# marcinmiklitz/pywindow

Hardware: AMD Instinct MI355X
Metric: trajectory frames/sec full_analysis (pore+windows), CC3 1k-frame (higher is better)
Workload: dtype f64

## Files before the change

### pywindow_amd/csrc/pw_lbfgsb.hpp

```cpp
#pragma once
#include "pw_blas.hpp"
#include "pw_team.hpp"

#if defined(PW_PROFILE) && defined(__HIP_DEVICE_COMPILE__)
#define LB_T0(var) long long var = wall_clock64()
#define LB_T1(slot, var) do { if (prof && T::lane() == 0) atomicAdd(&prof[slot], (unsigned long long)(wall_clock64() - var)); } while (0)
#else
#define LB_T0(var) do {} while (0)
#define LB_T1(slot, var) do {} while (0)
#endif
#if defined(PW_PROFILE) && defined(PW_LB_FINE) && defined(__HIP_DEVICE_COMPILE__)
#define LB_F0(var) long long var = clock64()
#define LB_F1(slot, var) do { if (prof && T::lane() == 0) atomicAdd(&prof[slot], (unsigned long long)(clock64() - var)); } while (0)
#define LB_M0(var) long long var = clock64()
#define LB_M1(slot, var) do { if (m->prof_fine && T::lane() == 0) atomicAdd(&m->prof_fine[slot], (unsigned long long)(clock64() - var)); } while (0)
#else
#define LB_F0(var) do {} while (0)
#define LB_F1(slot, var) do {} while (0)
#define LB_M0(var) do {} while (0)
#define LB_M1(slot, var) do {} while (0)
#endif

namespace pw {

enum LbTask : int {
    LB_START = 0,
    LB_NEW_X = 1,
    LB_FG = 3,
    LB_CONVERGENCE = 4,
    LB_STOP = 5,
    LB_WARNING = 6,
    LB_ERROR = 7,
    LB_ABNORMAL = 8,
};
enum LbMsg : int {
    LBM_NONE = 0,
    LBM_FG_START = 301,
    LBM_FG_LNSRCH = 302,
    LBM_CONV_PGTOL = 401,
    LBM_CONV_FTOL = 402,
};

constexpr int LB_M = 10;

struct LsState {
    double ginit, gtest, gx, gy, finit, fx, fy, stx, sty, stmin, stmax, width, width1;
    int brackt, stage;
};

template <int N>
struct LbMem {
    static constexpr int M = LB_M;
    static constexpr int M2 = 2 * LB_M;
    double l[N], u[N];
    double x[N], g[N];
    double ws[M * N], wy[M * N];
    double sy[M * M], ss[M * M], wt[M * M];
    double wn[M2 * M2], wn1d[M2];
    double z[N], r[N], d[N], t[N], xp[N];
    double wa[8 * M];
    double acc[2 * M];
    double dsy[M], rsy[M], sqy[M], rsq[M], rwt[M], rwn[M2];
    double iwn[M];
    double tri[64];
    int pair[64];
    double le[N], ue[N];
    LsState ls;
#if defined(PW_PROFILE) && defined(PW_LB_FINE)
    unsigned long long* prof_fine;
#endif
    int cand[32];
    int nbd[N];
    int index[N], iwhere[N], indx2[N];
};

template <class T>
PW_NOINLINE PW_HD inline void lb_trsv_un_wave(int n, const double* a, int lda, double* x) {
    PW_ASSUME_LDS(a);
    PW_ASSUME_LDS(x);
    const int lane = T::lane();
    double xk = lane < n ? x[lane] : 0.0;
    for (int i = n - 1; i >= 0; --i) {
        const double* ci = a + (long)i * lda;
        double xi = T::bcast_u(xk, i) / ci[i];
        if (lane == i) xk = xi;
        if (lane < i) xk = pw_fma(-xi, ci[lane], xk);
    }
    T::wave_sync();
    if (lane < n) x[lane] = xk;
    T::wave_sync();
}
template <class T>
PW_NOINLINE PW_HD inline void lb_trsv_ut_wave(int n, const double* a, int lda, double* x) {
    PW_ASSUME_LDS(a);
    PW_ASSUME_LDS(x);
    const int lane = T::lane();
    const double* ci = a + (long)(lane < n ? lane : 0) * lda;
    double xk = lane < n ? x[lane] : 0.0;
    double ak = 0.0;
    for (int s = 0; s < n; ++s) {
        double xs = T::bcast_u(xk, s);
        if (s > 0) xs = xs - T::bcast_u(ak, s);
        xs = xs / a[s + (long)s * lda];
        if (lane == s) xk = xs;
        if (lane > s && lane < n) {
            if (lane >= 16 && s < 16) {
                if (s == 15) {
                    double sl[4];
                    for (int l = 0; l < 4; ++l) {
                        double a0 = ci[l] * T::bcast_u(xk, l);
                        double a1 = ci[4 + l] * T::bcast_u(xk, 4 + l);
                        double a2 = ci[8 + l] * T::bcast_u(xk, 8 + l);
                        double a3 = ci[12 + l] * T::bcast_u(xk, 12 + l);
                        sl[l] = ((a0 + a1) + a2) + a3;
                    }
                    ak = (sl[0] + sl[2]) + (sl[1] + sl[3]);
                }
            } else {
                ak = pw_fma(xs, ci[s], ak);
            }
        }
    }
    T::wave_sync();
    if (lane < n) x[lane] = xk;
    T::wave_sync();
}


#if defined(__HIP_DEVICE_COMPILE__)
typedef DeviceTeam<1> LbWave;
__device__ inline int lb_uniform(int v) { return __builtin_amdgcn_readfirstlane(v); }
template <class P>
__device__ inline P* lb_uniform(P* p) {
    union { P* p; int i[2]; } a;
    a.p = p;
    a.i[0] = __builtin_amdgcn_readfirstlane(a.i[0]);
    a.i[1] = __builtin_amdgcn_readfirstlane(a.i[1]);
    return a.p;
}
template <class T, int NMAX, bool SPEC>
__device__ inline __attribute__((always_inline)) double lb_solve_ut_reg(int n, const double* a, int lda, const double* rdiag,
                                                                       double xk, double* tnum) {
    PW_ASSUME_LDS(a);
    PW_ASSUME_LDS(rdiag);
    const int lane = T::lane();
    const bool act = lane < n;
    const int li = act ? lane : 0;
    const double* ci = a + li * lda;
    double c[NMAX];
#pragma unroll
    for (int k = 0; k < NMAX; ++k) c[k] = ci[k];
    int dli = li * (lda + 1);
    asm volatile("" : "+v"(dli));
    double dg = a[dli], rd = rdiag[li];
    if (!act) { dg = 1.0; rd = 1.0; xk = 0.0; }
    const double x0 = xk;
    double ak = 0.0;
#pragma unroll
    for (int s = 0; s < NMAX; ++s) {
        if (s >= n) continue;
        const double mine = SPEC ? pw_div_ru(xk - ak, dg, rd) : pw_div_r(xk - ak, dg, rd);
        const double xs = T::bcast_u(mine, s);
        xk = lane == s ? xs : xk;
        if (NMAX > 16 && s < 16) {
            if (s == 15) {
                double sl[4];
#pragma unroll
                for (int l = 0; l < 4; ++l) {
                    double a0 = c[l] * T::bcast_u(xk, l);
                    double a1 = c[4 + l] * T::bcast_u(xk, 4 + l);
                    double a2 = c[8 + l] * T::bcast_u(xk, 8 + l);
                    double a3 = c[12 + l] * T::bcast_u(xk, 12 + l);
                    sl[l] = ((a0 + a1) + a2) + a3;
                }
                const double blk = (sl[0] + sl[2]) + (sl[1] + sl[3]);
                ak = (act && lane >= 16) ? blk : ak;
            }
            ak = (act && lane > s && lane < 16) ? pw_fma(xs, c[s], ak) : ak;
        } else {
            ak = (act && lane > s) ? pw_fma(xs, c[s], ak) : ak;
        }
    }
    if (SPEC) *tnum = act ? x0 - ak : 1.0;
    return xk;
}
template <class T, int NMAX, bool SPEC>
__device__ inline __attribute__((always_inline)) double lb_solve_un_reg(int n, const double* a, int lda, const double* rdiag,
                                                                       double xk, double* tnum) {
    PW_ASSUME_LDS(a);
    PW_ASSUME_LDS(rdiag);
    const int lane = T::lane();
    const bool act = lane < n;
    const int li = act ? lane : 0;
    double rw[NMAX];
#pragma unroll
    for (int i = 0; i < NMAX; ++i) rw[i] = a[li + i * lda];
    int dli = li * (lda + 1);
    asm volatile("" : "+v"(dli));
    double dg = a[dli], rd = rdiag[li];
    if (!act) { dg = 1.0; rd = 1.0; xk = 0.0; }
    double tn = 1.0;
#pragma unroll
    for (int i = NMAX - 1; i >= 0; --i) {
        if (i >= n) continue;
        const double mine = SPEC ? pw_div_ru(xk, dg, rd) : pw_div_r(xk, dg, rd);
        const double xi = T::bcast_u(mine, i);
        if (SPEC) tn = lane == i ? xk : tn;
        xk = lane == i ? xi : xk;
        xk = lane < i ? pw_fma(-xi, rw[i], xk) : xk;
    }
    if (SPEC) *tnum = tn;
    return xk;
}
__device__ inline unsigned lb_expo(double x) {
    union { double d; unsigned long long u; } c;
    c.d = x;
    return (unsigned)(c.u >> 32) & 0x7ff00000u;
}
__device__ inline bool lb_plain_range(unsigned emin, unsigned emax) {
    return (emin - 0x2bc00000u) <= 0x2bc00000u && (emax - 0x2bc00000u) <= 0x2bc00000u;
}

template <class T, int N, bool SPEC>
__device__ inline __attribute__((always_inline)) int lb_bmv_body(LbMem<N>* m, int col, const double* v, double* p) {
    constexpr int M = LB_M;
    const int lane = T::lane();
    const bool act = lane < col;
    const int li = act ? lane : 0;
    {
        const unsigned long long z = T::ballot(act && m->wt[li + M * li] == 0.0);
        if (z) return (int)__builtin_ctzll(z) + 1;
    }
    LB_M0(tb0);
    const double vi = act ? v[li] : 0.0, vc = act ? v[col + li] : 0.0;
    unsigned emin = 0x3ff00000u, emax = 0x3ff00000u;
    const int pk = m->pair[lane];
    const int pa_ = pk & 0xff, pb_ = (pk >> 8) & 0xff;
    const bool pact = pa_ < col;
    const int sa = pact ? pa_ : 1, sb = pact ? pb_ : 0;
    const double sy_ab = m->sy[sa + M * sb], d_b = m->dsy[sb], r_b = m->rsy[sb];
    {
        const double num = pact ? sy_ab * v[sb] : 1.0;
        if (SPEC) {
            const unsigned e = lb_expo(num);
            emin = e < emin ? e : emin;
            emax = e > emax ? e : emax;
        }
        const double term = SPEC ? pw_div_ru(num, d_b, r_b) : pw_div_r(num, d_b, r_b);
        m->tri[lane] = term;
    }
    T::wave_sync();
    double sum = 0.0;
    {
        const int base = li * (li - 1) / 2;
        double q[M - 1];
#pragma unroll
        for (int k = 0; k < M - 1; ++k) q[k] = m->tri[(base + k) & 63];
#pragma unroll
        for (int k = 0; k < M - 1; ++k) {
            const bool on = act && k < lane && k + 1 < col;
            sum = sum + (on ? q[k] : 0.0);
        }
    }
    double xk = lane == 0 ? vc : vc + sum;
    double t_ut = 1.0, t_un = 1.0;
    LB_M1(3, tb0);
    LB_M0(tb1);
    xk = lb_solve_ut_reg<T, M, SPEC>(col, m->wt, M, m->rwt, xk, &t_ut);
    LB_M1(4, tb1);
    LB_M0(tb2);
    const double sq = act ? m->sqy[li] : 1.0, rs = act ? m->rsq[li] : 1.0;
    const double pa = SPEC ? pw_div_ru(vi, sq, rs) : pw_div_r(vi, sq, rs);
    xk = lb_solve_un_reg<T, M, SPEC>(col, m->wt, M, m->rwt, xk, &t_un);
    LB_M1(5, tb2);
    LB_M0(tb3);
    const double pi = SPEC ? pw_div_ru(-pa, sq, rs) : pw_div_r(-pa, sq, rs);
    if (act) p[col + lane] = xk;
    T::wave_sync();
    {
        const double num = pact ? sy_ab * p[col + sa] : 1.0;
        if (SPEC) {
            const unsigned e = lb_expo(num);
            emin = e < emin ? e : emin;
            emax = e > emax ? e : emax;
        }
        const double term = SPEC ? pw_div_ru(num, d_b, r_b) : pw_div_r(num, d_b, r_b);
        m->tri[lane] = term;
    }
    T::wave_sync();
    double sum2 = 0.0;
    {
        double q[M];
#pragma unroll
        for (int k = 1; k < M; ++k) q[k] = m->tri[(k * (k - 1) / 2 + li) & 63];
#pragma unroll
        for (int k = 1; k < M; ++k) {
            const bool on = act && k > lane && k < col;
            sum2 = sum2 + (on ? q[k] : 0.0);
        }
    }
    if (SPEC) {
        unsigned e;
        e = lb_expo(t_ut); emin = e < emin ? e : emin; emax = e > emax ? e : emax;
        e = lb_expo(t_un); emin = e < emin ? e : emin; emax = e > emax ? e : emax;
        if (act) {
            e = lb_expo(vi); emin = e < emin ? e : emin; emax = e > emax ? e : emax;
            e = lb_expo(pa); emin = e < emin ? e : emin; emax = e > emax ? e : emax;
        }
        bool good = lb_plain_range(emin, emax) && rs != 0.0 && (!pact || r_b != 0.0) && (!act || m->rwt[li] != 0.0);
        if (T::ballot(!good)) return -1;
    }
    if (act) p[lane] = pi + sum2;
    T::wave_sync();
    LB_M1(6, tb3);
    return 0;
}
template <class T, int N>
PW_NOINLINE __device__ inline int lb_bmv_wave_guarded(LbMem<N>* m, int col, const double* v, double* p) {
    m = lb_uniform(m); v = lb_uniform(v); p = lb_uniform(p); col = lb_uniform(col);
    PW_ASSUME_LDS(m);
    PW_ASSUME_LDS(v);
    PW_ASSUME_LDS(p);
    return lb_bmv_body<T, N, false>(m, col, v, p);
// ... 1132 lines not shown
            WN1(iy, jy) = WN1(iy, jy) + temp1 - temp3;
            WN1(is, js) = WN1(is, js) - temp2 + temp4;
        }
        for (int e = T::lane(); e < upcl * upcl; e += T::WSIZE) {
            int ii = e / upcl, jy = e % upcl;
            int is = M + ii;
            int ipntr = (head + ii) % M, jpntr = (head + jy) % M;
            double temp1 = 0.0, temp3 = 0.0;
            for (int k = 0; k < nenter; ++k) {
                int k1 = indx2[k];
                temp1 = temp1 + WS(ipntr)[k1] * WY(jpntr)[k1];
            }
            for (int k = ileave - 1; k < N; ++k) {
                int k1 = indx2[k];
                temp3 = temp3 + WS(ipntr)[k1] * WY(jpntr)[k1];
            }
            if (is <= jy + M) WN1(is, jy) = WN1(is, jy) + temp1 - temp3;
            else WN1(is, jy) = WN1(is, jy) - temp1 + temp3;
        }
        }
        T::wave_sync();
        for (int e = T::lane(); e < col * col; e += T::WSIZE) {
            int iy = e / col, jy = e % col;
            int is = col + iy, is1 = M + iy;
            if (jy <= iy) {
                int js = col + jy, js1 = M + jy;
                double w = WN1(iy, jy) / theta;
                if (jy == iy) w = w + SY(iy, iy);
                WN(jy, iy) = w;
                WN(js, is) = WN1(is1, js1) * theta;
            }
            if (jy < iy) WN(jy, is) = -WN1(is1, jy);
            else WN(jy, is) = WN1(is1, jy);
        }
        T::wave_sync();
        LB_F1(8, fk1);
        if (col <= 2) {
            LB_F0(fks);
            const int rs = formk_tail_small<T>();
            LB_F1(9, fks);
            return rs;
        }
        LB_F0(fk2);
        int inf = factor<T>(2);
        LB_F1(9, fk2);
        if (inf != 0) return -1;
        int col2 = 2 * col;
        LB_F0(fk3);
#if defined(__HIP_DEVICE_COMPILE__)
        inf = p_dtrtrs_u<T>(true, col, col, wn, M2, &WN(0, col), M2, T::WSIZE == 64 ? mem->iwn : (const double*)nullptr);
#else
        inf = p_dtrtrs_u<T>(true, col, col, wn, M2, &WN(0, col), M2);
#endif
        LB_F1(10, fk3);
        LB_F0(fk4);
        for (int e = T::lane(); e < col * col; e += T::WSIZE) {
            int is = col + e / col, js = col + e % col;
            if (js < is) continue;
            WN(is, js) = WN(is, js) + b_ddot(col, &WN(0, is), &WN(0, js));
        }
        T::wave_sync();
        inf = factor<T>(3);
        LB_F1(11, fk4);
        (void)col2;
        if (inf != 0) return -2;
        return 0;
    }

    template <class T>
    PW_HD int cmprlb() {
        PW_ASSUME_LDS(mem);
        if (!cnstnd && col > 0) {
            for (int i = 0; i < N; ++i) r[i] = -g[i];
        } else {
            for (int i = 0; i < nfree; ++i) {
                int k = index[i];
                r[i] = -theta * (z[k] - x[k]) - g[k];
            }
            T::wave_sync();
            int inf = bmv<T>(wa + 2 * M, wa);
            if (inf != 0) return -8;
            LB_F0(fr);
#if defined(__HIP_DEVICE_COMPILE__)
            if (T::WSIZE == 64) {
                const int lj = T::lane();
                const bool lon = lj < col;
                const int pj = (head + (lon ? lj : 0)) % M;
                const double a1 = lon ? wa[lj] : 0.0, a2 = lon ? theta * wa[col + lj] : 0.0;
                double t1[N], t2[N], rl[N];
                for (int i = 0; i < N; ++i) {
                    const int k = i < nfree ? index[i] : 0;
                    t1[i] = WY(pj)[k] * a1;
                    t2[i] = WS(pj)[k] * a2;
                    rl[i] = r[i];
                }
#pragma unroll
                for (int jj = 0; jj < M; ++jj) {
                    if (jj >= col) continue;
#pragma unroll
                    for (int i = 0; i < N; ++i)
                        if (i < nfree) rl[i] = rl[i] + T::bcast_u(t1[i], jj) + T::bcast_u(t2[i], jj);
                }
                T::wave_sync();
                for (int i = 0; i < N; ++i)
                    if (i < nfree) r[i] = rl[i];
                T::wave_sync();
            } else
#endif
            {
                int pointr = head;
                for (int j = 0; j < col; ++j) {
                    double a1 = wa[j];
                    double a2 = theta * wa[col + j];
                    for (int i = 0; i < nfree; ++i) {
                        int k = index[i];
                        r[i] = r[i] + WY(pointr)[k] * a1 + WS(pointr)[k] * a2;
                    }
                    pointr = (pointr + 1) % M;
                }
            }
            LB_F1(13, fr);
        }
        return 0;
    }

    template <class T>
    PW_HD int subsm() {
        PW_ASSUME_LDS(mem);
        const int nsub = nfree;
        double* wv = wa;
        double* dd = r;
        double* xs = z;
        if (nsub <= 0) return 0;
        T::wave_sync();
        LB_F0(fsh);
        for (int i = T::lane(); i < col; i += T::WSIZE) {
            int pi = (head + i) % M;
            double temp1 = 0.0, temp2 = 0.0;
            for (int j = 0; j < nsub; ++j) {
                int k = index[j];
                temp1 = temp1 + WY(pi)[k] * dd[j];
                temp2 = temp2 + WS(pi)[k] * dd[j];
            }
            wv[i] = temp1;
            wv[col + i] = theta * temp2;
        }
        T::wave_sync();
        LB_F1(29, fsh);
        int col2 = 2 * col;
        LB_F0(fs1);
        int inf;
        if (col <= 2) {
            inf = subsm_solves_small<T>(wv);
        } else
#if defined(__HIP_DEVICE_COMPILE__)
        if (T::WSIZE == 64) {
            inf = lb_subsm_solves_wave<LbWave, N>(mem, col, wv);
        } else
#endif
        {
            inf = p_dtrtrs_u<T>(true, col2, 1, wn, M2, wv, col2);
            if (inf != 0) return inf;
            for (int i = T::lane(); i < col; i += T::WSIZE) wv[i] = -wv[i];
            T::wave_sync();
            inf = p_dtrtrs_u<T>(false, col2, 1, wn, M2, wv, col2);
        }
        LB_F1(12, fs1);
        if (inf != 0) return inf;
        LB_F0(fst);
        if (T::WSIZE == 64 && col * nsub <= 32) {
            const int t = T::lane();
            const int nsu = T::uniform_i(nsub), cu = T::uniform_i(col);
            const int jy_ = nsu == 3 ? t / 3 : (nsu == 2 ? t >> 1 : t), i_ = t - jy_ * nsu;
            const double rth = 1.0 / theta;
            if (jy_ < cu) {
                const int pj = (head + jy_) % M, k = index[i_];
                mem->tri[t] = WY(pj)[k] * wv[jy_] / theta;
                mem->tri[32 + t] = WS(pj)[k] * wv[cu + jy_];
            }
            double acc_[N];
            for (int i = 0; i < N; ++i) acc_[i] = dd[i < nsu ? i : 0];
            T::wave_sync();
            double q1[M * N], q2[M * N];
#pragma unroll
            for (int jy = 0; jy < M; ++jy)
#pragma unroll
                for (int i = 0; i < N; ++i) {
                    const int at = (jy * nsu + i) & 31;
                    q1[jy * N + i] = mem->tri[at];
                    q2[jy * N + i] = mem->tri[32 + at];
                }
#pragma unroll
            for (int jy = 0; jy < M; ++jy)
#pragma unroll
                for (int i = 0; i < N; ++i) {
                    const bool on = jy < cu && i < nsu;
                    acc_[i] = acc_[i] + (on ? q1[jy * N + i] : -0.0) + (on ? q2[jy * N + i] : -0.0);
                }
            T::wave_sync();
            for (int i = 0; i < N; ++i)
                if (i < nsu) dd[i] = rth * acc_[i];
            T::wave_sync();
        } else {
            int pointr = head;
            for (int jy = 0; jy < col; ++jy) {
                int js = col + jy;
                for (int i = 0; i < nsub; ++i) {
                    int k = index[i];
                    dd[i] = dd[i] + WY(pointr)[k] * wv[jy] / theta + WS(pointr)[k] * wv[js];
                }
                pointr = (pointr + 1) % M;
            }
            b_dscal(nsub, 1.0 / theta, dd);
        }
        iword = 0;
        b_dcopy(N, xs, xp);
        {
            int kk[N], nb[N];
            double dk[N], xk[N], lk[N], uk[N];
            for (int i = 0; i < N; ++i) {
                const bool on = i < nsub;
                kk[i] = on ? index[i] : 0;
            }
            for (int i = 0; i < N; ++i) {
                dk[i] = dd[i < nsub ? i : 0]; xk[i] = xs[kk[i]]; nb[i] = nbd[kk[i]]; lk[i] = l[kk[i]]; uk[i] = u[kk[i]];
            }
            T::wave_sync();
            for (int i = 0; i < N; ++i) {
                if (i >= nsub) continue;
                double nx;
                bool hit = false;
                if (nb[i] != 0) {
                    nx = xk[i];
                    if (nb[i] == 1) {
                        nx = pw_max(lk[i], xk[i] + dk[i]);
                        hit = nx == lk[i];
                    } else if (nb[i] == 2) {
                        nx = pw_min(uk[i], pw_max(lk[i], xk[i] + dk[i]));
                        hit = nx == lk[i] || nx == uk[i];
                    } else if (nb[i] == 3) {
                        nx = pw_min(uk[i], xk[i] + dk[i]);
                        hit = nx == uk[i];
                    }
                } else {
                    nx = xk[i] + dk[i];
                }
                if (hit) iword = 1;
                xs[kk[i]] = nx;
            }
            T::wave_sync();
        }
        LB_F1(30, fst);
        if (iword == 0) return 0;
        double dd_p = 0.0;
        for (int i = 0; i < N; ++i) dd_p = dd_p + (xs[i] - x[i]) * g[i];
        if (dd_p > 0.0) {
            b_dcopy(N, xp, xs);
            double alpha = 1.0;
            double temp1 = alpha;
            int ibd = 0;
            for (int i = 0; i < nsub; ++i) {
                int k = index[i];
                double dk = dd[i];
                if (nbd[k] != 0) {
                    if (dk < 0.0 && nbd[k] <= 2) {
                        double temp2 = l[k] - xs[k];
                        if (temp2 >= 0.0) temp1 = 0.0;
                        else if (dk * alpha < temp2) temp1 = temp2 / dk;
                    } else if (dk > 0.0 && nbd[k] >= 2) {
                        double temp2 = u[k] - xs[k];
                        if (temp2 <= 0.0) temp1 = 0.0;
                        else if (dk * alpha > temp2) temp1 = temp2 / dk;
                    }
                    if (temp1 < alpha) {
                        alpha = temp1;
                        ibd = i;
                    }
                }
            }
            if (alpha < 1.0) {
                double dk = dd[ibd];
                int k = index[ibd];
                if (dk > 0.0) {
                    xs[k] = u[k];
                    dd[ibd] = 0.0;
                } else if (dk < 0.0) {
                    xs[k] = l[k];
                    dd[ibd] = 0.0;
                }
            }
            for (int i = 0; i < nsub; ++i) {
                int k = index[i];
                xs[k] = xs[k] + alpha * dd[i];
            }
        }
        return 0;
    }

    template <class T>
    PW_HD bool lnsrlb(bool reentry) {
        PW_ASSUME_LDS(mem);
        const double big = 1.0e10, ftol = 1.0e-3, gtol = 0.9, xtol = 0.1;
        if (!reentry) {
            dnorm = b_dnrm2(N, d);
            dtd = dnorm * dnorm;
            stpmx = big;
            if (cnstnd) {
                if (iter == 0) {
                    stpmx = 1.0;
                } else {
                    for (int i = 0; i < N; ++i) {
                        double a1 = d[i];
                        if (nbd[i] != 0) {
                            if (a1 < 0.0 && nbd[i] <= 2) {
                                double a2 = l[i] - x[i];
                                if (a2 >= 0.0) stpmx = 0.0;
                                else if (a1 * stpmx < a2) stpmx = a2 / a1;
                            } else if (a1 > 0.0 && nbd[i] >= 2) {
                                double a2 = u[i] - x[i];
                                if (a2 <= 0.0) stpmx = 0.0;
                                else if (a1 * stpmx > a2) stpmx = a2 / a1;
                            }
                        }
                    }
                }
            }
            if (iter == 0 && !boxed) stp = pw_min(1.0 / dnorm, stpmx);
            else stp = 1.0;
            b_dcopy(N, x, t);
            b_dcopy(N, g, r);
            fold = f;
            ifun = 0;
            iback = 0;
            ls_task = 0;
        }
        gd = b_ddot(N, g, d);
        if (ifun == 0) {
            gdold = gd;
            if (gd >= 0.0) {
                info = -4;
                return false;
            }
        }
        LB_F0(fl);
        {
            const LsOut o = lb_dcsrch(&mem->ls, ls_task, f, gd, stp, ftol, gtol, xtol, 0.0, stpmx);
            stp = o.st;
            ls_task = o.task;
        }
        LB_F1(23, fl);
        if (ls_task != 2 && ls_task != 3) {
            task = LB_FG;
            msg = LBM_FG_LNSRCH;
            ifun += 1;
            nfgv += 1;
            iback = ifun - 1;
            if (stp == 1.0) {
                b_dcopy(N, z, x);
            } else {
                for (int i = 0; i < N; ++i) x[i] = pw_min(pw_max(stp * d[i] + t[i], mem->le[i]), mem->ue[i]);
            }
            return true;
        }
        task = LB_NEW_X;
        msg = 0;
        return false;
    }

    template <class T>
    PW_HD void matupd(double rr, double dr) {
        PW_ASSUME_LDS(mem);
        if (iupdat <= M) {
            col = iupdat;
            itail = (head + iupdat - 1) % M;
        } else {
            itail = (itail + 1) % M;
            head = (head + 1) % M;
        }
        b_dcopy(N, d, WS(itail));
        b_dcopy(N, r, WY(itail));
        theta = rr / dr;
        T::wave_sync();
        if (iupdat > M) {
            constexpr int PERM = ((M - 1) * (M - 1) + T::WSIZE - 1) / T::WSIZE;
            double keep_ss[PERM], keep_sy[PERM];
            int cnt = (col - 1) * (col - 1);
#pragma unroll
            for (int q = 0; q < PERM; ++q) {
                keep_ss[q] = keep_sy[q] = 0.0;
                int e = T::lane() + q * T::WSIZE;
                if (e < cnt && T::WSIZE > 1) {
                    int j = e / (col - 1), i = e % (col - 1);
                    keep_ss[q] = (i <= j) ? SS(i + 1, j + 1) : 0.0;
                    keep_sy[q] = (i >= j) ? SY(i + 1, j + 1) : 0.0;
                }
            }
            if (T::WSIZE > 1) {
                T::wave_sync();
#pragma unroll
                for (int q = 0; q < PERM; ++q) {
                    int e = T::lane() + q * T::WSIZE;
                    if (e < cnt) {
                        int j = e / (col - 1), i = e % (col - 1);
                        if (i <= j) SS(i, j) = keep_ss[q];
                        if (i >= j) SY(i, j) = keep_sy[q];
                    }
                }
            } else {
                for (int j = 0; j < col - 1; ++j) {
                    b_dcopy(j + 1, &SS(1, j + 1), &SS(0, j));
                    b_dcopy(col - (j + 1), &SY(j + 1, j + 1), &SY(j, j));
                }
            }
            T::wave_sync();
        }
        for (int j = T::lane(); j < col - 1; j += T::WSIZE) {
            int pj = (head + j) % M;
            SY(col - 1, j) = b_ddot(N, d, WY(pj));
            SS(j, col - 1) = b_ddot(N, WS(pj), d);
        }
        if (T::lane() == 0) {
            if (stp == 1.0) SS(col - 1, col - 1) = dtd;
            else SS(col - 1, col - 1) = stp * stp * dtd;
            SY(col - 1, col - 1) = dr;
        }
        T::wave_sync();
        tables<T>(0);
    }

    template <class T>
    PW_HD int formt() {
        PW_ASSUME_LDS(mem);
        if (col <= 2) {
            double w00 = theta * SS(0, 0), w01 = 0.0, w11 = 0.0;
            int inf;
            if (col == 1) {
                inf = potf2_1(w00);
            } else {
                w01 = theta * SS(0, 1);
                const double ddum = 0.0 + SY(1, 0) * SY(1, 0) / SY(0, 0);
                w11 = ddum + theta * SS(1, 1);
                inf = potf2_2(w00, w01, w11);
            }
            T::wave_sync();
            WT(0, 0) = w00;
            if (col == 2) { WT(0, 1) = w01; WT(1, 1) = w11; }
            T::wave_sync();
            return inf != 0 ? -3 : 0;
        }
        for (int e = T::lane(); e < col * col; e += T::WSIZE) {
            int i = e / col, j = e % col;
            if (j < i) continue;
            if (i == 0) {
                WT(0, j) = theta * SS(0, j);
            } else {
                double ddum = 0.0;
                for (int k = 0; k < i; ++k) ddum = ddum + SY(i, k) * SY(j, k) / SY(k, k);
                WT(i, j) = ddum + theta * SS(i, j);
            }
        }
        T::wave_sync();
        int inf = factor<T>(1);
        if (inf != 0) return -3;
        return 0;
    }

    PW_HD void refresh() {
        info = 0;
        col = 0;
        head = 0;
        theta = 1.0;
        iupdat = 0;
        updatd = false;
    }

    template <class T, class FG>
    PW_HD __attribute__((always_inline)) bool linesearch(FG& fg) {
        PW_ASSUME_LDS(mem);
        LB_F0(fh);
        const double big = 1.0e10, ftol = 1.0e-3, gtol = 0.9, xtol = 0.1;
        double dv[N], xv[N], zv[N], gv[N], tv[N], lev[N], uev[N];
        int nbv[N];
        for (int i = 0; i < N; ++i) {
            dv[i] = d[i]; xv[i] = x[i]; zv[i] = z[i]; gv[i] = g[i]; lev[i] = mem->le[i]; uev[i] = mem->ue[i]; nbv[i] = nbd[i];
        }
        dnorm = b_dnrm2(N, d);
        dtd = dnorm * dnorm;
        stpmx = big;
        if (cnstnd) {
            if (iter == 0) {
                stpmx = 1.0;
            } else {
                for (int i = 0; i < N; ++i) {
                    double a1 = dv[i];
                    if (nbv[i] != 0) {
                        if (a1 < 0.0 && nbv[i] <= 2) {
                            double a2 = l[i] - xv[i];
                            if (a2 >= 0.0) stpmx = 0.0;
                            else if (a1 * stpmx < a2) stpmx = a2 / a1;
                        } else if (a1 > 0.0 && nbv[i] >= 2) {
                            double a2 = u[i] - xv[i];
                            if (a2 <= 0.0) stpmx = 0.0;
                            else if (a1 * stpmx > a2) stpmx = a2 / a1;
                        }
                    }
                }
            }
        }
        if (iter == 0 && !boxed) stp = pw_min(1.0 / dnorm, stpmx);
        else stp = 1.0;
        for (int i = 0; i < N; ++i) { tv[i] = xv[i]; t[i] = xv[i]; r[i] = gv[i]; }
        fold = f;
        ifun = 0;
        iback = 0;
        ls_task = 0;
        LsState L = LsState{};
        bool ok;
        LB_F1(26, fh);
        for (;;) {
            double dot = 0.0;
            for (int i = 0; i < N; ++i) dot = pw_fma(dv[i], gv[i], dot);
            gd = dot;
            if (ifun == 0) {
                gdold = gd;
                if (gd >= 0.0) { info = -4; ok = false; break; }
            }
            LB_F0(fl);
            {
                const LsOut o = lb_dcsrch_core(L, ls_task, f, gd, stp, ftol, gtol, xtol, 0.0, stpmx);
                stp = o.st;
                ls_task = o.task;
            }
            LB_F1(23, fl);
            if (ls_task == 2 || ls_task == 3) {
                task = LB_NEW_X;
                msg = 0;
                ok = true;
                break;
            }
            task = LB_FG;
            msg = LBM_FG_LNSRCH;
            ifun += 1;
            nfgv += 1;
            iback = ifun - 1;
            if (stp == 1.0) {
                for (int i = 0; i < N; ++i) xv[i] = zv[i];
            } else {
                for (int i = 0; i < N; ++i) xv[i] = pw_min(pw_max(stp * dv[i] + tv[i], lev[i]), uev[i]);
            }
            if (iback >= maxls) { ok = false; break; }
            LB_F0(fe);
            fg(xv, f, gv);
            LB_F1(25, fe);
        }
        if (ok) {
            for (int i = 0; i < N; ++i) { x[i] = xv[i]; g[i] = gv[i]; }
        } else {
            for (int i = 0; i < N; ++i) { x[i] = tv[i]; g[i] = r[i]; }
            f = fold;
        }
        T::wave_sync();
        return ok;
    }

    template <class T, class FG>
    PW_HD __attribute__((always_inline)) void minimize(FG& fg, int maxiter, int maxfun, int* nit_out) {
        PW_ASSUME_LDS(mem);
        int nit = 0;
        *nit_out = 0;
        epsmch = 2.220446049250313e-16;
        col = 0; head = 0; theta = 1.0; iupdat = 0; updatd = false;
        iback = 0; itail = 0; iword = 0; nact = 0; ileave = 0; nenter = 0;
        fold = 0.0; dnorm = 0.0; gd = 0.0; stpmx = 0.0; sbgnrm = 0.0; stp = 0.0;
        gdold = 0.0; dtd = 0.0;
        iter = 0; nfgv = 0; nseg = 0; nintol = 0; nskip = 0; nfree = N; ifun = 0;
        tol = factr * epsmch;
        info = 0;
        ls_task = 0;
        for (int i = 0; i < N; ++i) { index[i] = 0; indx2[i] = 0; }
        active();
        task = LB_FG;
        msg = LBM_FG_START;
        T::wave_sync();
        {
            double xv[N], gv[N];
            for (int i = 0; i < N; ++i) xv[i] = x[i];
            fg(xv, f, gv);
            for (int i = 0; i < N; ++i) g[i] = gv[i];
            T::wave_sync();
        }
        nfgv = 1;
        projgr();
        if (sbgnrm <= pgtol) {
            task = LB_CONVERGENCE;
            msg = LBM_CONV_PGTOL;
            return;
        }
        for (;;) {
            iword = -1;
            bool wrk;
            if (!cnstnd && col > 0) {
                b_dcopy(N, x, z);
                wrk = updatd;
                nseg = 0;
            } else {
                LB_T0(tc);
                int inf = cauchy<T>();
                LB_T1(16, tc);
                if (inf != 0) { refresh(); continue; }
                nintol += nseg;
                wrk = freev();
                nact = N - nfree;
            }
            if (!(nfree == 0 || col == 0)) {
                if (wrk) {
                    LB_T0(tk);
                    int inf = formk<T>();
                    LB_T1(17, tk);
                    if (inf != 0) { refresh(); continue; }
                }
                LB_T0(tm);
                int inf = cmprlb<T>();
                LB_T1(18, tm);
                LB_T0(tsb);
                if (inf == 0) inf = subsm<T>();
                LB_T1(19, tsb);
                if (inf != 0) { refresh(); continue; }
            }
            for (int i = 0; i < N; ++i) d[i] = z[i] - x[i];
            T::wave_sync();
            LB_T0(tl);
            const bool newx = linesearch<T>(fg);
            LB_T1(20, tl);
            if (!newx) {
                if (col == 0) {
                    if (info == 0) {
                        info = -9;
                        nfgv -= 1;
                        ifun -= 1;
                        iback -= 1;
                    }
                    task = LB_ABNORMAL;
                    msg = 0;
                    iter += 1;
                    *nit_out = nit;
                    return;
                }
                if (info == 0) nfgv -= 1;
                refresh();
                continue;
            }
            iter += 1;
            projgr();
            nit += 1;
            *nit_out = nit;
            if (nit >= maxiter || fg.nfev > maxfun) return;
            if (sbgnrm <= pgtol) {
                task = LB_CONVERGENCE;
                msg = LBM_CONV_PGTOL;
                return;
            }
            double ddum = pw_max(pw_max(pw_abs(fold), pw_abs(f)), 1.0);
            if ((fold - f) <= tol * ddum) {
                task = LB_CONVERGENCE;
                msg = LBM_CONV_FTOL;
                if (iback >= 10) info = -5;
                return;
            }
            for (int i = 0; i < N; ++i) r[i] = g[i] - r[i];
            double rr = b_dnrm2(N, r);
            rr = rr * rr;
            double dr;
            if (stp == 1.0) {
                dr = gd - gdold;
                ddum = -gdold;
            } else {
                dr = (gd - gdold) * stp;
                b_dscal(N, stp, d);
                ddum = -gdold * stp;
            }
            if (dr <= epsmch * ddum) {
                nskip += 1;
                updatd = false;
                continue;
            }
            updatd = true;
            iupdat += 1;
            LB_T0(tu);
            matupd<T>(rr, dr);
            LB_T1(21, tu);
            LB_T0(tf);
            int inf = formt<T>();
            LB_T1(22, tf);
            if (inf != 0) { refresh(); continue; }
        }
    }

    template <class T>
    PW_HD void step() {
        PW_ASSUME_LDS(mem);
        int entry;
        if (task == LB_START) {
            epsmch = 2.220446049250313e-16;
            col = 0; head = 0; theta = 1.0; iupdat = 0; updatd = false;
            iback = 0; itail = 0; iword = 0; nact = 0; ileave = 0; nenter = 0;
            fold = 0.0; dnorm = 0.0; gd = 0.0; stpmx = 0.0; sbgnrm = 0.0; stp = 0.0;
            gdold = 0.0; dtd = 0.0;
            iter = 0; nfgv = 0; nseg = 0; nintol = 0; nskip = 0; nfree = N; ifun = 0;
            tol = factr * epsmch;
            info = 0;
            for (int i = 0; i < N; ++i) { index[i] = 0; indx2[i] = 0; }
            active();
            task = LB_FG;
            msg = LBM_FG_START;
            return;
        } else if (task == LB_FG && msg == LBM_FG_START) {
            entry = 1;
        } else if (task == LB_FG) {
            entry = 2;
        } else if (task == LB_NEW_X) {
            entry = 3;
        } else {
            return;
        }

        if (entry == 1) {
            nfgv = 1;
            projgr();
            if (sbgnrm <= pgtol) {
                task = LB_CONVERGENCE;
                msg = LBM_CONV_PGTOL;
                return;
            }
        }
        bool resume_ls = (entry == 2);
        bool resume_newx = (entry == 3);
        for (;;) {
            if (!resume_ls && !resume_newx) {
                iword = -1;
                bool wrk;
                bool have_dir = false;
                if (!cnstnd && col > 0) {
                    b_dcopy(N, x, z);
                    wrk = updatd;
                    nseg = 0;
                } else {
                    LB_T0(tc);
                    int inf = cauchy<T>();
                    LB_T1(16, tc);
                    if (inf != 0) { refresh(); continue; }
                    nintol += nseg;
                    wrk = freev();
                    nact = N - nfree;
                }
                if (!(nfree == 0 || col == 0)) {
                    if (wrk) {
                        LB_T0(tk);
                        int inf = formk<T>();
                        LB_T1(17, tk);
                        if (inf != 0) { refresh(); continue; }
                    }
                    LB_T0(tm);
                    int inf = cmprlb<T>();
                    LB_T1(18, tm);
                    LB_T0(tsb);
                    if (inf == 0) inf = subsm<T>();
                    LB_T1(19, tsb);
                    if (inf != 0) { refresh(); continue; }
                }
                (void)have_dir;
                for (int i = 0; i < N; ++i) d[i] = z[i] - x[i];
            }
            if (!resume_newx) {
                LB_T0(tl);
                bool need_fg = lnsrlb<T>(resume_ls);
                LB_T1(20, tl);
                resume_ls = false;
                if (info != 0 || iback >= maxls) {
                    b_dcopy(N, t, x);
                    b_dcopy(N, r, g);
                    f = fold;
                    if (col == 0) {
                        if (info == 0) {
                            info = -9;
                            nfgv -= 1;
                            ifun -= 1;
                            iback -= 1;
                        }
                        task = LB_ABNORMAL;
                        msg = 0;
                        iter += 1;
                        return;
                    } else {
                        if (info == 0) nfgv -= 1;
                        refresh();
                        continue;
                    }
                } else if (need_fg) {
                    return;
                } else {
                    iter += 1;
                    projgr();
                    return;
                }
            }
            resume_newx = false;
            if (sbgnrm <= pgtol) {
                task = LB_CONVERGENCE;
                msg = LBM_CONV_PGTOL;
                return;
            }
            double ddum = pw_max(pw_max(pw_abs(fold), pw_abs(f)), 1.0);
            if ((fold - f) <= tol * ddum) {
                task = LB_CONVERGENCE;
                msg = LBM_CONV_FTOL;
                if (iback >= 10) info = -5;
                return;
            }
            for (int i = 0; i < N; ++i) r[i] = g[i] - r[i];
            double rr = b_dnrm2(N, r);
            rr = rr * rr;
            double dr;
            if (stp == 1.0) {
                dr = gd - gdold;
                ddum = -gdold;
            } else {
                dr = (gd - gdold) * stp;
                b_dscal(N, stp, d);
                ddum = -gdold * stp;
            }
            if (dr <= epsmch * ddum) {
                nskip += 1;
                updatd = false;
                continue;
            }
            updatd = true;
            iupdat += 1;
            LB_T0(tu);
            matupd<T>(rr, dr);
            LB_T1(21, tu);
            LB_T0(tf);
            int inf = formt<T>();
            LB_T1(22, tf);
            if (inf != 0) { refresh(); continue; }
        }
    }
};

}
```

Baseline: 1.011 million.

## Add scalar fast path for one-variable L-BFGS-B direction and first update

```diff
diff --git a/pywindow_amd/csrc/pw_lbfgsb.hpp b/pywindow_amd/csrc/pw_lbfgsb.hpp
--- a/pywindow_amd/csrc/pw_lbfgsb.hpp
+++ b/pywindow_amd/csrc/pw_lbfgsb.hpp
@@ -19,6 +19,35 @@
 #define LB_F1(slot, var) do {} while (0)
 #define LB_M0(var) do {} while (0)
 #define LB_M1(slot, var) do {} while (0)
+#endif
+
+#if defined(PW_LB_STATS) && !defined(__HIP_DEVICE_COMPILE__) && !defined(__HIPCC__)
+namespace pw {
+enum LbStat : int {
+    LBS_STRAIGHT = 0,
+    LBS_DECLINED,
+    LBS_GENERIC,
+    LBS_UPDATE1,
+    LBS_LS_MORE,
+    LBS_LS_REFRESH,
+    LBS_LS_ABNORMAL,
+    LBS_NIT0, LBS_NIT1, LBS_NIT2, LBS_NIT3, LBS_NIT4,
+    LBS_END_LOWER, LBS_END_UPPER,
+    LBS_START_NONZERO,
+    LBS_NBD0, LBS_NBD1, LBS_NBD2, LBS_NBD3,
+    LBS_COUNT
+};
+static long lb_stats[LBS_COUNT];
+}
+#define LB_STAT(k) do { if (N == 1) ++pw::lb_stats[pw::k]; } while (0)
+#define LB_STAT_END(nit) do { if (N == 1) {                                                                       \
+        ++pw::lb_stats[pw::LBS_NIT0 + ((nit) < 4 ? (nit) : 4)];                                                   \
+        if ((nbd[0] == 1 || nbd[0] == 2) && x[0] == l[0]) ++pw::lb_stats[pw::LBS_END_LOWER];                      \
+        if ((nbd[0] == 2 || nbd[0] == 3) && x[0] == u[0]) ++pw::lb_stats[pw::LBS_END_UPPER];                      \
+    } } while (0)
+#else
+#define LB_STAT(k) do {} while (0)
+#define LB_STAT_END(nit) do {} while (0)
 #endif
 
 namespace pw {
@@ -1757,7 +1786,7 @@
         PW_ASSUME_LDS(mem);
         const double big = 1.0e10, ftol = 1.0e-3, gtol = 0.9, xtol = 0.1;
         if (!reentry) {
-            dnorm = b_dnrm2(N, d);
+            dnorm = nrm2_(d);
             dtd = dnorm * dnorm;
             stpmx = big;
             if (cnstnd) {
@@ -1920,6 +1949,16 @@
         return 0;
     }
 
+    PW_HD static double nrm2_(const double* v) {
+#if !defined(PW_LB_NO_STRAIGHT)
+        if constexpr (N == 1) {
+            const double a = pw_abs(v[0]);
+            if (a < PW_INF) return a;
+        }
+#endif
+        return b_dnrm2(N, v);
+    }
+
     PW_HD void refresh() {
         info = 0;
         col = 0;
@@ -1928,6 +1967,253 @@
         iupdat = 0;
         updatd = false;
     }
+
+#if !defined(PW_LB_NO_STRAIGHT)
+    PW_HD static int bmv_one_(double sy00, double w00, double v0, double v1, double& p0, double& p1) {
+        if (w00 == 0.0) return 1;
+        const double q0 = pw_sqrt(sy00);
+        double t1 = v1 / w00;
+        const double t0 = v0 / q0;
+        t1 = t1 / w00;
+        const double pi0 = -t0 / q0;
+        p0 = pi0 + 0.0;
+        p1 = t1;
+        return 0;
+    }
+    template <class T>
+    PW_HD __attribute__((always_inline)) bool direction1() {
+        static_assert(N == 1, "one variable");
+        PW_ASSUME_LDS(mem);
+        if (col > 1 || head != 0 || !(sbgnrm > 0.0)) return false;
+        const bool one = col == 1;
+        const bool run_cauchy = cnstnd || !one;
+        const double x0 = x[0], g0 = g[0], l0 = l[0], u0 = u[0], th = theta;
+        const int nb = nbd[0];
+        int iw = iwhere[0];
+        double wy0 = 0.0, ws0 = 0.0, sy00 = 0.0, w00 = 0.0;
+        if (one) { wy0 = wy[0]; ws0 = ws[0]; sy00 = SY(0, 0); w00 = WT(0, 0); }
+        double z0 = x0;
+        int nseg_n = nseg, nfree_n = nfree, nact_n = nact, nenter_n = nenter, ileave_n = ileave;
+        bool wrk = updatd;
+        bool wr_c = false;
+        double P0 = 0.0, P1 = 0.0;
+        double C0 = 0.0, C1 = 0.0;
+        double V0 = 0.0, V1 = 0.0;
+        if (run_cauchy) {
+            double tl = 0.0, tu = 0.0, f1 = 0.0, bkmin = 0.0, dl;
+            int nbreak = 0;
+            bool nofree = true;
+            const double neggi = -g0;
+            if (iw != 3 && iw != -1) {
+                if (nb <= 2) tl = x0 - l0;
+                if (nb >= 2) tu = u0 - x0;
+                const bool xlower = nb <= 2 && tl <= 0.0;
+                const bool xupper = nb >= 2 && tu <= 0.0;
+                iw = 0;
+                if (xlower) {
+                    if (neggi <= 0.0) iw = 1;
+                } else if (xupper) {
+                    if (neggi >= 0.0) iw = 2;
+                } else {
+                    if (pw_abs(neggi) <= 0.0) iw = -3;
+                }
+            }
+            double pa0 = 0.0, pb0 = 0.0;
+            if (iw != 0 && iw != -1) {
+                dl = 0.0;
+            } else {
+                dl = neggi;
+                f1 = f1 - neggi * neggi;
+                if (one) { pa0 = pa0 + wy0 * neggi; pb0 = pb0 + ws0 * neggi; }
+                if (nb <= 2 && nb != 0 && neggi < 0.0) {
+                    nbreak = 1;
+                    bkmin = tl / (-neggi);
+                } else if (nb >= 2 && neggi > 0.0) {
+                    nbreak = 1;
+                    bkmin = tu / neggi;
+                } else {
+                    nofree = false;
+                }
+            }
+            if (th != 1.0) pb0 = th * pb0;
+            P0 = pa0; P1 = pb0;
+            if (!(nbreak == 0 && nofree)) {
+                wr_c = one;
+                double f2 = -th * f1;
+                if (one) {
+                    if (bmv_one_(sy00, w00, P0, P1, V0, V1) != 0) return false;
+                    f2 = f2 - pw_fma(P1, V1, pw_fma(P0, V0, 0.0));
+                }
+                double dtm = -f1 / f2;
+                double tsum = 0.0;
+                nseg_n = 1;
+                bool at_999 = false;
+                if (nbreak != 0) {
+                    const double dt = bkmin - 0.0;
+                    if (!(dtm < dt)) {
+                        tsum = tsum + dt;
+                        if (dl > 0.0) { z0 = u0; iw = 2; }
+                        else { z0 = l0; iw = 1; }
+                        dl = 0.0;
+                        dtm = dt;
+                        at_999 = true;
+                    }
+                }
+                if (!at_999) {
+                    if (dtm <= 0.0) dtm = 0.0;
+                    tsum = tsum + dtm;
+                    z0 = pw_fma(tsum, dl, z0);
+                }
+                if (one) { C0 = pw_fma(dtm, P0, 0.0); C1 = pw_fma(dtm, P1, 0.0); }
+            }
+            nenter_n = 0;
+            ileave_n = N + 1;
+            if (iter > 0 && cnstnd) {
+                if (nfree >= 1) { if (iw > 0) ileave_n = N; }
+                else { if (iw <= 0) nenter_n = 1; }
+            }
+            wrk = (ileave_n < N + 1) || (nenter_n > 0) || updatd;
+            nfree_n = iw <= 0 ? 1 : 0;
+            nact_n = N - nfree_n;
+        }
+        const bool sub = one && nfree_n != 0;
+        double n11 = 0.0, n21 = 0.0, a00 = 0.0, a01 = 0.0, a11 = 0.0;
+        double W0 = 0.0, W1 = 0.0;
+        double xp0 = 0.0;
+        int iword_n = -1;
+        if (sub) {
+            if (run_cauchy && !wr_c) return false;
+            if (wrk) {
+                if (!updatd || nenter_n > 0 || ileave_n <= N) return false;
+                n11 = 0.0 + wy0 * wy0;
+                n21 = 0.0 + ws0 * wy0;
+                a00 = n11 / th + sy00;
+                a11 = 0.0 * th;
+                a01 = n21;
+                if (potf2_1(a00) != 0) return false;
+                if (a00 != 0.0) a01 = a01 / a00;
+                a11 = a11 + pw_fma(a01, a01, 0.0);
+                if (potf2_1(a11) != 0) return false;
+            } else {
+                a00 = WN(0, 0); a01 = WN(0, 1); a11 = WN(1, 1);
+            }
+            double r0;
+            if (!cnstnd) {
+                r0 = -g0;
+            } else {
+                r0 = -th * (z0 - x0) - g0;
+                double q0 = 0.0, q1 = 0.0;
+                if (bmv_one_(sy00, w00, C0, C1, q0, q1) != 0) return false;
+                r0 = r0 + wy0 * q0 + ws0 * (th * q1);
+            }
+            W0 = 0.0 + wy0 * r0;
+            W1 = th * (0.0 + ws0 * r0);
+            if (a00 == 0.0 || a11 == 0.0) return false;
+            W0 = W0 / a00;
+            W1 = (W1 - pw_fma(W0, a01, 0.0)) / a11;
+            W0 = -W0;
+            W1 = W1 / a11;
+            W0 = pw_fma(-W1, a01, W0);
+            W0 = W0 / a00;
+            r0 = r0 + wy0 * W0 / th + ws0 * W1;
+            r0 = (1.0 / th) * r0;
+            iword_n = 0;
+            xp0 = z0;
+            {
+                double nx;
+                bool hit = false;
+                if (nb != 0) {
+                    nx = z0;
+                    if (nb == 1) {
+                        nx = pw_max(l0, z0 + r0);
+                        hit = nx == l0;
+                    } else if (nb == 2) {
+                        nx = pw_min(u0, pw_max(l0, z0 + r0));
+                        hit = nx == l0 || nx == u0;
+                    } else if (nb == 3) {
+                        nx = pw_min(u0, z0 + r0);
+                        hit = nx == u0;
+                    }
+                } else {
+                    nx = z0 + r0;
+                }
+                if (hit) iword_n = 1;
+                z0 = nx;
+            }
+            if (iword_n != 0) {
+                double dd_p = 0.0;
+                dd_p = dd_p + (z0 - x0) * g0;
+                if (dd_p > 0.0) {
+                    z0 = xp0;
+                    double alpha = 1.0, temp1 = alpha;
+                    if (nb != 0) {
+                        if (r0 < 0.0 && nb <= 2) {
+                            const double temp2 = l0 - z0;
+                            if (temp2 >= 0.0) temp1 = 0.0;
+                            else if (r0 * alpha < temp2) temp1 = temp2 / r0;
+                        } else if (r0 > 0.0 && nb >= 2) {
+                            const double temp2 = u0 - z0;
+                            if (temp2 <= 0.0) temp1 = 0.0;
+                            else if (r0 * alpha > temp2) temp1 = temp2 / r0;
+                        }
+                        if (temp1 < alpha) alpha = temp1;
+                    }
+                    if (alpha < 1.0) {
+                        if (r0 > 0.0) { z0 = u0; r0 = 0.0; }
+                        else if (r0 < 0.0) { z0 = l0; r0 = 0.0; }
+                    }
+                    z0 = z0 + alpha * r0;
+                }
+            }
+        }
+        iword = iword_n;
+        if (run_cauchy) {
+            iwhere[0] = iw;
+            if (one) {
+                wa[0] = P0; wa[1] = P1;
+                if (wr_c) { wa[2 * M] = C0; wa[2 * M + 1] = C1; wa[6 * M] = V0; wa[6 * M + 1] = V1; }
+            }
+            nintol += nseg_n;
+            nfree = nfree_n;
+            nact = nact_n;
+            nenter = nenter_n;
+            ileave = ileave_n;
+            nseg = nseg_n;
+        } else {
+            nseg = 0;
+        }
+        if (sub) {
+            if (wrk) {
+                WN1(0, 0) = n11; WN1(M, M) = 0.0; WN1(M, 0) = n21;
+                WN(0, 0) = a00; WN(0, 1) = a01; WN(1, 1) = a11;
+            }
+            wa[0] = W0; wa[1] = W1;
+            xp[0] = xp0;
+        }
+        z[0] = z0;
+        d[0] = z0 - x0;
+        return true;
+    }
+    template <class T>
+    PW_HD __attribute__((always_inline)) int update1(double rr, double dr) {
+        static_assert(N == 1, "one variable");
+        PW_ASSUME_LDS(mem);
+        const double d0 = d[0], r0 = r[0];
+        col = 1;
+        itail = 0;
+        theta = rr / dr;
+        double sdiag;
+        if (stp == 1.0) sdiag = dtd;
+        else sdiag = stp * stp * dtd;
+        double w00 = theta * sdiag;
+        const int inf = potf2_1(w00);
+        ws[0] = d0; wy[0] = r0;
+        SS(0, 0) = sdiag; SY(0, 0) = dr;
+        WT(0, 0) = w00;
+        T::wave_sync();
+        return inf != 0 ? -3 : 0;
+    }
+#endif
 
     template <class T, class FG>
     PW_HD __attribute__((always_inline)) bool linesearch(FG& fg) {
@@ -1939,7 +2225,7 @@
         for (int i = 0; i < N; ++i) {
             dv[i] = d[i]; xv[i] = x[i]; zv[i] = z[i]; gv[i] = g[i]; lev[i] = mem->le[i]; uev[i] = mem->ue[i]; nbv[i] = nbd[i];
         }
-        dnorm = b_dnrm2(N, d);
+        dnorm = nrm2_(d);
         dtd = dnorm * dnorm;
         stpmx = big;
         if (cnstnd) {
@@ -2037,6 +2323,8 @@
         task = LB_FG;
         msg = LBM_FG_START;
         T::wave_sync();
+        LB_STAT(LBS_NBD0 + nbd[0]);
+        if (x[0] != 0.0) LB_STAT(LBS_START_NONZERO);
         {
             double xv[N], gv[N];
             for (int i = 0; i < N; ++i) xv[i] = x[i];
@@ -2049,9 +2337,20 @@
         if (sbgnrm <= pgtol) {
             task = LB_CONVERGENCE;
             msg = LBM_CONV_PGTOL;
+            LB_STAT_END(0);
             return;
         }
         for (;;) {
+#if !defined(PW_LB_NO_STRAIGHT)
+            if constexpr (N == 1) {
+                LB_T0(ts);
+                const bool straight = direction1<T>();
+                LB_T1(16, ts);
+                if (straight) { LB_STAT(LBS_STRAIGHT); goto have_direction; }
+            }
+#endif
+            if (col <= 1) LB_STAT(LBS_DECLINED);
+            else LB_STAT(LBS_GENERIC);
             iword = -1;
             bool wrk;
             if (!cnstnd && col > 0) {
@@ -2083,10 +2382,14 @@
                 if (inf != 0) { refresh(); continue; }
             }
             for (int i = 0; i < N; ++i) d[i] = z[i] - x[i];
+#if !defined(PW_LB_NO_STRAIGHT)
+        have_direction:
+#endif
             T::wave_sync();
             LB_T0(tl);
             const bool newx = linesearch<T>(fg);
             LB_T1(20, tl);
+            if (ifun > 1) LB_STAT(LBS_LS_MORE);
             if (!newx) {
                 if (col == 0) {
                     if (info == 0) {
@@ -2099,9 +2402,12 @@
                     msg = 0;
                     iter += 1;
                     *nit_out = nit;
+                    LB_STAT(LBS_LS_ABNORMAL);
+                    LB_STAT_END(nit);
                     return;
                 }
                 if (info == 0) nfgv -= 1;
+                LB_STAT(LBS_LS_REFRESH);
                 refresh();
                 continue;
             }
@@ -2109,10 +2415,11 @@
             projgr();
             nit += 1;
             *nit_out = nit;
-            if (nit >= maxiter || fg.nfev > maxfun) return;
+            if (nit >= maxiter || fg.nfev > maxfun) { LB_STAT_END(nit); return; }
             if (sbgnrm <= pgtol) {
                 task = LB_CONVERGENCE;
                 msg = LBM_CONV_PGTOL;
+                LB_STAT_END(nit);
                 return;
             }
             double ddum = pw_max(pw_max(pw_abs(fold), pw_abs(f)), 1.0);
@@ -2120,10 +2427,11 @@
                 task = LB_CONVERGENCE;
                 msg = LBM_CONV_FTOL;
                 if (iback >= 10) info = -5;
+                LB_STAT_END(nit);
                 return;
             }
             for (int i = 0; i < N; ++i) r[i] = g[i] - r[i];
-            double rr = b_dnrm2(N, r);
+            double rr = nrm2_(r);
             rr = rr * rr;
             double dr;
             if (stp == 1.0) {
@@ -2141,6 +2449,18 @@
             }
             updatd = true;
             iupdat += 1;
+#if !defined(PW_LB_NO_STRAIGHT)
+            if constexpr (N == 1) {
+                if (iupdat == 1 && head == 0) {
+                    LB_T0(tu1);
+                    const int inf1 = update1<T>(rr, dr);
+                    LB_T1(21, tu1);
+                    LB_STAT(LBS_UPDATE1);
+                    if (inf1 != 0) refresh();
+                    continue;
+                }
+            }
+#endif
             LB_T0(tu);
             matupd<T>(rr, dr);
             LB_T1(21, tu);
@@ -2191,7 +2511,13 @@
         bool resume_ls = (entry == 2);
         bool resume_newx = (entry == 3);
         for (;;) {
-            if (!resume_ls && !resume_newx) {
+            bool straight = false;
+#if !defined(PW_LB_NO_STRAIGHT)
+            if constexpr (N == 1) {
+                if (!resume_ls && !resume_newx) straight = direction1<T>();
+            }
+#endif
+            if (!resume_ls && !resume_newx && !straight) {
                 iword = -1;
                 bool wrk;
                 bool have_dir = false;
@@ -2273,7 +2599,7 @@
                 return;
             }
             for (int i = 0; i < N; ++i) r[i] = g[i] - r[i];
-            double rr = b_dnrm2(N, r);
+            double rr = nrm2_(r);
             rr = rr * rr;
             double dr;
             if (stp == 1.0) {
@@ -2291,6 +2617,17 @@
             }
             updatd = true;
             iupdat += 1;
+#if !defined(PW_LB_NO_STRAIGHT)
+            if constexpr (N == 1) {
+                if (iupdat == 1 && head == 0) {
+                    LB_T0(tu1);
+                    const int inf1 = update1<T>(rr, dr);
+                    LB_T1(21, tu1);
+                    if (inf1 != 0) refresh();
+                    continue;
+                }
+            }
+#endif
             LB_T0(tu);
             matupd<T>(rr, dr);
             LB_T1(21, tu);
```

Result: no change. 1.012 million (median of 2 runs) (+0.1%).
